# SciLifeLab/TIDDIT

Measured on AMD Instinct MI355X. Metric: cov bins/sec, 30x WGS synthetic (signals clustered/sec: see 'dbscan'), higher is better.
Workload: dtype int64; 1 GPU; BASELINE configs[1]: coverage histogram, 24 contigs x 125000000 bp (3.00 Gb), 30x 150-bp sorted stream, 500-bp bins, q>=20 filter; contigs split over the 1 rank(s); reads=600000000, bins=6000000

## Files before the change

### tiddit_amd/csrc/tdt_coverage.hip

```cpp
extern const char *const tdt_variant_coverage;
const char *const tdt_variant_coverage = ""
#ifdef COV_MIN_WAVES
    " COV_MIN_WAVES"
#endif
#ifdef COV_MIN_WAVES1
    " COV_MIN_WAVES1"
#endif
#ifdef COV_MIN_WAVES1_4
    " COV_MIN_WAVES1_4"
#endif
#ifdef COV_MIN_WAVES4
    " COV_MIN_WAVES4"
#endif
#ifdef COV_RPL
    " COV_RPL"
#endif
#ifdef COV_RPL1
    " COV_RPL1"
#endif
#ifdef COV_SPARES1
    " COV_SPARES1"
#endif
#ifdef COV_WIN
    " COV_WIN"
#endif
#ifdef COV_WIN1
    " COV_WIN1"
#endif
    ;

#include "tdt_common.h"

#include <algorithm>
#include <thread>

#define COV_THREADS 256
#ifndef COV_RPL
#define COV_RPL 8
#endif
#ifndef COV_RPL1
#define COV_RPL1 4
#endif
#define COV_READS_PER_BLOCK 16384
#ifndef COV_WIN
#define COV_WIN 2048
#endif
#define COV_LUT_LDS_MAX 1024
#define COV_PUSH_CHUNK (4u << 20)
#define COV_STATUS_BYTES (128 + COV_KEPT_SLOTS * 128)
#define COV_KEPT_SLOTS 512

struct CovItem {
    const int32_t *start;
    const int32_t *end;
    const uint8_t *mapq;
    const uint16_t *flag;
    const unsigned long long *packed;
    unsigned long long n;
    unsigned long long *acc;
    const unsigned long long *lut_end;
    int nbins;
    int aligned;
    unsigned first_block;
    unsigned binned;
};

struct CovParams {
    CovItem it;
    const CovItem *items;
    int n_items;
    int bin_size;
    unsigned magic;
    int shift;
    int min_q;
    int margin;
    unsigned xmax, m15;
    int k15;
    const unsigned long long *lut_main;
    unsigned long long one;
    int *status;
    unsigned long long *kept;
};

__device__ __forceinline__ int cov_div(int x, unsigned magic, int shift) {
    return shift < 0 ? x : (int)(__umulhi((unsigned)x, magic) >> shift);
}

#define DPP_WAVE_SHL1 0x130
#define DPP_WAVE_SHR1 0x138

template <int CTRL>
__device__ __forceinline__ unsigned long long dpp_u64(unsigned long long v) {
    const unsigned lo = __builtin_amdgcn_update_dpp(0u, (unsigned)v, CTRL, 0xf, 0xf, true);
    const unsigned hi = __builtin_amdgcn_update_dpp(0u, (unsigned)(v >> 32), CTRL, 0xf, 0xf, true);
    return ((unsigned long long)hi << 32) | lo;
}

#define COV_DPP_SHR1 "row_shr:1 row_mask:0xf bank_mask:0xf bound_ctrl:0"
#define COV_DPP_SHR2 "row_shr:2 row_mask:0xf bank_mask:0xf bound_ctrl:0"
#define COV_DPP_SHR4 "row_shr:4 row_mask:0xf bank_mask:0xf bound_ctrl:0"
#define COV_DPP_SHR8 "row_shr:8 row_mask:0xf bank_mask:0xf bound_ctrl:0"
#define COV_DPP_BC15 "row_bcast:15 row_mask:0xa bank_mask:0xf"
#define COV_DPP_BC31 "row_bcast:31 row_mask:0xc bank_mask:0xf"
#define COV_SCAN_ALL(STEP) \
    "s_nop 1\n\t" STEP(COV_DPP_SHR1) STEP(COV_DPP_SHR2) STEP(COV_DPP_SHR4) STEP(COV_DPP_SHR8) STEP(COV_DPP_BC15) STEP(COV_DPP_BC31) "s_nop 1"
#define COV_SCAN_STEP(CTRL)                                                                     \
    "v_add_co_u32_dpp %0, vcc, %0, %0 " CTRL "\n\t"                                             \
    "v_addc_co_u32_dpp %1, vcc, %1, %1, vcc " CTRL "\n\t"                                       \
    "v_add_co_u32_dpp %2, vcc, %2, %2 " CTRL "\n\t"                                             \
    "v_addc_co_u32_dpp %3, vcc, %3, %3, vcc " CTRL "\n\t"                                       \
    "v_add_co_u32_dpp %4, vcc, %4, %4 " CTRL "\n\t"                                             \
    "v_addc_co_u32_dpp %5, vcc, %5, %5, vcc " CTRL "\n\t"

__device__ __forceinline__ void wave_scan3_u64(unsigned long long &a0, unsigned long long &a1, unsigned long long &a2) {
    unsigned l0 = (unsigned)a0, h0 = (unsigned)(a0 >> 32), l1 = (unsigned)a1, h1 = (unsigned)(a1 >> 32),
             l2 = (unsigned)a2, h2 = (unsigned)(a2 >> 32);
    asm volatile(COV_SCAN_ALL(COV_SCAN_STEP) : "+v"(l0), "+v"(h0), "+v"(l1), "+v"(h1), "+v"(l2), "+v"(h2)::"vcc", "memory");
    a0 = ((unsigned long long)h0 << 32) | l0;
    a1 = ((unsigned long long)h1 << 32) | l1;
    a2 = ((unsigned long long)h2 << 32) | l2;
}

__device__ __forceinline__ unsigned long long cov_mask_lt(unsigned a, unsigned lim_uniform) {
    unsigned long long m;
    asm("v_cmp_gt_u32_e64 %0, %1, %2" : "=s"(m) : "s"(lim_uniform), "v"(a));
    return m;
}
__device__ __forceinline__ unsigned long long cov_mask_eq0(unsigned a) {
    unsigned long long m;
    asm("v_cmp_eq_u32_e64 %0, 0, %1" : "=s"(m) : "v"(a));
    return m;
}
__device__ __forceinline__ unsigned long long cov_mask_ne0(unsigned a) {
    unsigned long long m;
    asm("v_cmp_ne_u32_e64 %0, 0, %1" : "=s"(m) : "v"(a));
    return m;
}
__device__ __forceinline__ unsigned cov_select(unsigned long long m, unsigned if_set, unsigned if_clear) {
    unsigned r;
    asm("v_cndmask_b32_e64 %0, %1, %2, %3" : "=v"(r) : "v"(if_clear), "v"(if_set), "s"(m));
    return r;
}

#define COV_SCAN2_STEP(CTRL)                                                                    \
    "v_add_co_u32_dpp %0, vcc, %0, %0 " CTRL "\n\t"                                             \
    "v_addc_co_u32_dpp %1, vcc, %1, %1, vcc " CTRL "\n\t"                                       \
    "v_add_co_u32_dpp %2, vcc, %2, %2 " CTRL "\n\t"                                             \
    "v_addc_co_u32_dpp %3, vcc, %3, %3, vcc " CTRL "\n\t"

__device__ __forceinline__ void wave_scan2_u64(unsigned long long &a0, unsigned long long &a1) {
    unsigned l0 = (unsigned)a0, h0 = (unsigned)(a0 >> 32), l1 = (unsigned)a1, h1 = (unsigned)(a1 >> 32);
    asm volatile(COV_SCAN_ALL(COV_SCAN2_STEP) : "+v"(l0), "+v"(h0), "+v"(l1), "+v"(h1)::"vcc", "memory");
    a0 = ((unsigned long long)h0 << 32) | l0;
    a1 = ((unsigned long long)h1 << 32) | l1;
}

#define COV_SCAN4I_STEP(CTRL)                                                                   \
    "v_add_u32_dpp %0, %0, %0 " CTRL "\n\t"                                                     \
    "v_add_u32_dpp %1, %1, %1 " CTRL "\n\t"                                                     \
    "v_add_u32_dpp %2, %2, %2 " CTRL "\n\t"                                                     \
    "v_add_u32_dpp %3, %3, %3 " CTRL "\n\t"

__device__ __forceinline__ void wave_scan4_i32(int &p0, int &p1, int &p2, int &p3) {
    asm volatile(COV_SCAN_ALL(COV_SCAN4I_STEP) : "+v"(p0), "+v"(p1), "+v"(p2), "+v"(p3)::"memory");
}
// ... 75 lines not shown
            t.mq[j / 4] |= (ok ? (unsigned)P.mapq[idx + j] : 0u) << (8 * (j & 3));
            t.fl[j / 2] |= (ok ? (unsigned)P.flag[idx + j] : 0x4u) << (16 * (j & 1));
        }
    }
    return t;
}

template <int RPL>
struct CovTileP {
    unsigned long long w[RPL];
};

template <int RPL>
__device__ __forceinline__ CovTileP<RPL> cov_load_packed(const CovItem &P, unsigned long long idx, unsigned long long r1) {
    CovTileP<RPL> t;
    if (P.aligned && idx + RPL <= r1) {
#pragma unroll
        for (int k = 0; k < RPL / 2; k++) {
            const ulonglong2 v = *reinterpret_cast<const ulonglong2 *>(P.packed + idx + 2 * k);
            t.w[2 * k] = v.x;
            t.w[2 * k + 1] = v.y;
        }
    } else {
#pragma unroll
        for (int j = 0; j < RPL; j++) t.w[j] = idx + j < r1 ? P.packed[idx + j] : (1ull << 62);
    }
    return t;
}

__global__ void cov_pack(const int32_t *__restrict__ start, const int32_t *__restrict__ end, const uint8_t *__restrict__ mapq,
                         const uint16_t *__restrict__ flag, unsigned long long n, unsigned long long *__restrict__ out) {
    unsigned long long i = (unsigned long long)blockIdx.x * blockDim.x + threadIdx.x;
    const unsigned long long stride = (unsigned long long)gridDim.x * blockDim.x;
    for (; i < n; i += stride) out[i] = cov_pack_record(start[i], end[i], mapq[i], flag[i]);
}

__global__ void cov_pack_binned(const int32_t *__restrict__ start, const int32_t *__restrict__ end, const uint8_t *__restrict__ mapq,
                                const uint16_t *__restrict__ flag, unsigned long long n, int nbins, unsigned z, unsigned magic, int shift, int mode1,
                                unsigned long long *__restrict__ out) {
    unsigned long long i = (unsigned long long)blockIdx.x * blockDim.x + threadIdx.x;
    const unsigned long long stride = (unsigned long long)gridDim.x * blockDim.x;
    for (; i < n; i += stride) out[i] = cov_bin_record(start[i], end[i], mapq[i], flag[i], nbins, z, magic, shift, mode1 != 0);
}

#define COV_DBIT 48
#define COV_LOWMASK ((1ull << COV_DBIT) - 1ull)
#ifndef COV_WIN1
#define COV_WIN1 2048
#endif
#define COV_DQMAX 256
#ifndef COV_SPARES1
#define COV_SPARES1 64
#endif

#ifndef COV_MIN_WAVES
#define COV_MIN_WAVES 4
#endif
#ifndef COV_MIN_WAVES4
#define COV_MIN_WAVES4 3
#endif
#ifndef COV_MIN_WAVES1
#define COV_MIN_WAVES1 6
#endif
#ifndef COV_MIN_WAVES1_4
#define COV_MIN_WAVES1_4 4
#endif
template <bool LDS_LUT, int MODE, bool Z1, int RPL, int REC>
__global__ __launch_bounds__(COV_THREADS, MODE == 1 ? (REC ? COV_MIN_WAVES1 : COV_MIN_WAVES1_4) : (REC ? COV_MIN_WAVES : COV_MIN_WAVES4)) void cov_accumulate(CovParams P) {
    constexpr bool PACKED = REC != 0;
    extern __shared__ __attribute__((aligned(16))) unsigned long long smem[];
    constexpr int WIN = MODE == 1 ? COV_WIN1 : COV_WIN;
    constexpr int TILE = COV_THREADS * RPL;
    int *s_wsum = reinterpret_cast<int *>(smem);
    int *s_tbin = s_wsum + 4;
    int *s_rtot = reinterpret_cast<int *>(smem + 12);
    unsigned long long *win = smem + 12 + (MODE == 1 ? 16 : 0);
    unsigned long long *lutS = win + WIN + (MODE == 1 ? COV_SPARES1 : 2);

    const int tid = threadIdx.x;
    const int lane = tid & 63;
    CovItem I = P.it;
    unsigned blk = blockIdx.x;
    if (P.n_items > 0) {
        int lo = 0, hi = P.n_items;
        while (hi - lo > 1) {
            const int mid = (lo + hi) >> 1;
            if (P.items[mid].first_block <= blk) lo = mid;
            else hi = mid;
        }
        I = P.items[lo];
        blk -= I.first_block;
    }
    const unsigned long long r0 = (unsigned long long)blk * COV_READS_PER_BLOCK;
    const unsigned long long r1 = min(I.n, r0 + COV_READS_PER_BLOCK);
    const unsigned z = (unsigned)P.bin_size;
    const int last_bin = I.nbins - 1;
    auto div = [&](int x) { return Z1 ? x : (int)(__umulhi((unsigned)x, P.magic) >> P.shift); };

    auto load_tile = [&](unsigned long long idx) {
        if constexpr (PACKED) return cov_load_packed<RPL>(I, idx, r1);
        else return cov_load<RPL>(I, idx, r1);
    };
    auto cur = load_tile(r0 + (unsigned long long)tid * RPL);

    for (int i = tid; i < WIN + 2; i += COV_THREADS) win[i] = 0;
    if (LDS_LUT) {
        for (unsigned i = tid; i <= z; i += COV_THREADS) {
            const unsigned long long v = P.lut_main[i];
            lutS[i] = v;
            lutS[i + z + 1] = I.lut_end[i];
            if (MODE == 0 && !Z1) {
                unsigned long long *pr = lutS + 2 * (z + 1);
                pr[2 * i] = v;
                pr[2 * i + 1] = 0;
                pr[2 * (z + 1) + 2 * i] = 0;
                pr[2 * (z + 1) + 2 * i + 1] = v;
            }
            if (MODE == 1) {
                unsigned long long *tabA = lutS + 2 * (z + 1), *tabB = tabA + (z + 1), *tabL = tabB + (z + 1);
                tabA[i] = v & 0xffffffffull;
                tabB[i] = v << 32;
                tabL[i] = v - (1ull << COV_DBIT);
                if (i == 0) tabL[z + 1] = 0;
            }
        }
    }
    auto bin_of_read = [&](unsigned long long idx) {
        if constexpr (REC == 2) return (int)((unsigned)I.packed[idx] >> 2);
        int s = PACKED ? (int)(unsigned)I.packed[idx] : I.start[idx];
        s = s < 0 ? 0 : s;
        const int b = div(s);
        return b < I.nbins ? b : I.nbins - 1;
    };
    if (tid < COV_READS_PER_BLOCK / TILE) {
        const unsigned long long tl = min(r0 + (unsigned long long)(tid + 1) * TILE, r1) - 1;
        s_tbin[tid] = bin_of_read(tl);
    }
    int base = bin_of_read(r0);
    __syncthreads();
    auto lut = [&](unsigned i) -> unsigned long long {
        if (LDS_LUT) return lutS[i];
        return i <= z ? P.lut_main[i] : I.lut_end[i - z - 1];
    };

    auto contribute = [&](int bin, unsigned long long v) {
        const unsigned off = (unsigned)(bin - base);
        if (off < (unsigned)WIN) atomicAdd(&win[off], v);
        else if ((unsigned)bin <= (unsigned)last_bin) cov_global_add(I.acc, bin, v);
    };

    auto slow_read = [&](int s, int e) {
        const int fb = div(s);
        const int eb = div(e - 1);
        if (fb == eb) {
            contribute(fb, lut((unsigned)(e - s)));
        } else {
            contribute(fb, lut((unsigned)(fb + 1) * z - (unsigned)s));
            const unsigned bl = (unsigned)(e - 1) - (unsigned)eb * z;
            contribute(eb, lut(eb < last_bin ? bl : bl + z + 1));
            for (int b = fb + 1; b < eb; b++) contribute(b, P.one);
        }
    };

    auto spill = [&]() {
        __syncthreads();
        if constexpr (MODE == 1) {
            constexpr int PER = WIN / COV_THREADS;
            static_assert(PER == 8 && COV_THREADS == 256, "the packed resolve is written for eight rows of 256 words");
            unsigned long long w[PER];
#pragma unroll
            for (int k = 0; k < PER; k++) w[k] = win[k * COV_THREADS + tid];
            int pk[PER / 2];
#pragma unroll
// ... 308 lines not shown
            const unsigned long long q0 = dpp_u64<DPP_WAVE_SHR1>(a0), q1 = dpp_u64<DPP_WAVE_SHR1>(a1), q2 = dpp_u64<DPP_WAVE_SHR1>(a2);
            if (Knext != K) {
                if (a0) contribute(K, a0);
                if (a1) contribute(K + 1, a1);
                if (a2) contribute(K + 2, a2);
            }
            if (Kprev != K && lane != 0) {
                if (q0) contribute(K, 0ull - q0);
                if (q1) contribute(K + 1, 0ull - q1);
                if (q2) contribute(K + 2, 0ull - q2);
            }
        } else {
            const unsigned long long *tabA = lutS + 2 * (z + 1), *tabL = tabA + 2 * (z + 1);
            const unsigned ko = (unsigned)(K - base);
            const bool safe = ko < (unsigned)(WIN - COV_DQMAX - 2) && K + COV_DQMAX + 2 <= last_bin;
            const unsigned kw = safe ? ko : 0u;
            unsigned d1 = 0, d2 = 0;
            unsigned long long vL[RPL];
            unsigned woff[RPL];
#pragma unroll
            for (int j = 0; j < RPL; j++) {
                const unsigned rs = (unsigned)sv[j] - Kz;
                const unsigned re1 = (unsigned)ev[j] - Kz;
                const unsigned len = re1 - rs;
                bool cand;
                if constexpr (PACKED) cand = (unsigned)(cur.w[j] >> 32) - ((unsigned)P.min_q << 24) < ((64u - (unsigned)P.min_q) << 24);
                else cand = ((fl[j] & FMASK) == 0) & ((int)mq[j] >= P.min_q);
                const bool fast = cand & safe & (rs < 2u * z) & (len - 1u < P.xmax) & (re1 <= P.xmax);
                nkept += fast ? 1u : 0u;
                slowmask |= (cand & !fast) ? (1u << j) : 0u;
                const bool r1_ = rs >= z;
                const unsigned dq = (__umul24(re1, P.m15) - P.m15) >> P.k15;
                const bool multi = fast & (dq != (r1_ ? 1u : 0u));
                const unsigned bf = min(len, (r1_ ? 2u * z : z) - rs);
                const unsigned long long vv = tabA[(fast ? bf : 0u) + (r1_ ? z + 1u : 0u)];
                a0 += (unsigned)vv;
                a1 += (unsigned)(vv >> 32);
                d1 += (multi & !r1_) ? 1u : 0u;
                d2 += (multi & r1_) ? 1u : 0u;
                const unsigned bl1 = re1 - __umul24(dq, z);
                vL[j] = tabL[multi ? bl1 - 1u : z + 1u];
                woff[j] = multi ? kw + dq : (unsigned)WIN;
            }
#pragma unroll
            for (int j = 0; j < RPL; j++) atomicAdd(&win[woff[j]], vL[j]);
            atomicAdd(&win[kw], a0);
            atomicAdd(&win[kw + 1], a1 + ((unsigned long long)d1 << COV_DBIT));
            atomicAdd(&win[kw + 2], (unsigned long long)d2 << COV_DBIT);
            if (slowmask) {
#pragma unroll
                for (int j = 0; j < RPL; j++)
                    if (slowmask & (1u << j)) {
                        const int s = sv[j], e = true_end(j);
                        if (s < 0 || e <= s || div(e - 1) > last_bin) bad = true;
                        else { nkept++; slow_read(s, e); }
                    }
            }
        }
        cur = nxt;
    }

    for (int d = 32; d > 0; d >>= 1) nkept += __shfl_down(nkept, d);
    nkept += nkept_s;
    if (lane == 0 && nkept)
        atomicAdd(P.kept + (size_t)((blockIdx.x * (COV_THREADS / 64) + (tid >> 6)) % COV_KEPT_SLOTS) * 16, (unsigned long long)nkept);
    if (bad) atomicOr(P.status, 1);

    spill();
}

__global__ void cov_finalize(const long long *__restrict__ acc, double *__restrict__ out, long long n, double inv_scale,
                             int *status) {
    long long i = (long long)blockIdx.x * blockDim.x + threadIdx.x;
    const long long stride = (long long)gridDim.x * blockDim.x;
    bool inexact = false;
    for (; i < n; i += stride) {
        const long long a = acc[i];
        if (a >= (1ll << 53) || a < 0) inexact = true;
        out[i] = (double)a * inv_scale;
    }
    if (inexact) atomicOr(status, 2);
}

struct tdt_cov {
    tdt_ctx *ctx = nullptr;
    int n_contigs = 0;
    int bin_size = 0;
    int S = 0;
    bool small_bins = false;
    unsigned xmax = 0, m15 = 0;
    int k15 = 0;
    unsigned magic = 0;
    int shift = 0;
    std::vector<int64_t> len, nbins, off;
    std::vector<int> end_bin_size;
    int64_t total_bins = 0;
    unsigned long long *d_acc = nullptr;
    unsigned long long *d_lut_main = nullptr;
    unsigned long long *d_lut_end = nullptr;
    int *d_status = nullptr;
    unsigned long long *d_kept = nullptr;
    int *d_nbins = nullptr;
    void *d_stage[2] = {nullptr, nullptr};
    void *h_stage[2] = {nullptr, nullptr};
    hipEvent_t slot_ev[2] = {nullptr, nullptr};
    int slot_used[2] = {0, 0};
    int next_slot = 0;
};

static bool build_lut(std::vector<unsigned long long> &lut, int bin_size, int den, int S) {
    const double scale = ldexp(1.0, S);
    for (int b = 0; b <= bin_size; b++) {
        volatile float q = (float)b / (float)den;
        double f = (double)q * scale;
        unsigned long long fx = (unsigned long long)f;
        if ((double)fx != f) return false;
        lut[b] = fx;
    }
    return true;
}

extern "C" int tdt_cov_create(tdt_ctx *ctx, const int64_t *contig_len, int n_contigs, int bin_size, tdt_cov **out) {
    if (!ctx || !contig_len || !out || n_contigs <= 0) {
        tdt_set_error("tdt_cov_create: bad argument");
        return TDT_E_ARG;
    }
    *out = nullptr;
    if (bin_size <= 0 || bin_size > (1 << 24)) {
        tdt_set_error("tdt_cov_create: bin_size %d outside [1, 2^24] (reference: float32 bases are exact only there)",
                      bin_size);
        return TDT_E_ARG;
    }
    TDT_HIP(hipSetDevice(ctx->device));
    tdt_cov *c = new tdt_cov();
    c->ctx = ctx;
    c->n_contigs = n_contigs;
    c->bin_size = bin_size;
    const int L = tdt_ceil_log2_u64((uint64_t)bin_size);
    c->S = 23 + L + 1;
    {
        const char *env = getenv("TIDDIT_COV_MODE");
        const bool can = bin_size >= 2 && c->S <= 31;
        c->small_bins = can;
        if (env && env[0] == '0') c->small_bins = false;
        if (bin_size >= 2 && bin_size + 1 <= COV_LUT_LDS_MAX) {
            c->k15 = 15 + L;
            c->m15 = (unsigned)(((1ull << c->k15) + (unsigned)bin_size - 1) / (unsigned)bin_size);
            const unsigned lim = (unsigned)COV_DQMAX * (unsigned)bin_size;
            c->xmax = lim < 32768u ? lim : 32768u;
            for (unsigned x = 0; x < 32768u; x++)
                if (((x * c->m15) >> c->k15) != x / (unsigned)bin_size) {
                    tdt_set_error("internal: 24-bit division self-check failed for d=%d x=%u", bin_size, x);
                    delete c;
                    return TDT_E_ARG;
                }
        }
    }
    if (L == 0) {
        c->shift = -1;
        c->magic = 0;
    } else {
        const unsigned __int128 num = (unsigned __int128)1 << (31 + L);
        const unsigned __int128 m = (num + (unsigned)bin_size - 1) / (unsigned)bin_size;
        c->magic = (unsigned)m;
        c->shift = L - 1;
        const int probes[] = {0, 1, bin_size - 1, bin_size, bin_size + 1, 2 * bin_size - 1, 2 * bin_size, 1000003,
                              0x3fffffff, 0x7ffffffe, 0x7fffffff};
        for (int x : probes) {
            if (x < 0) continue;
            const int q = (int)(((unsigned long long)(unsigned)x * c->magic) >> 32 >> c->shift);
            if (q != x / bin_size) {
                tdt_set_error("internal: magic division self-check failed for d=%d x=%d", bin_size, x);
                delete c;
                return TDT_E_ARG;
            }
        }
    }
    c->len.assign(contig_len, contig_len + n_contigs);
    c->nbins.resize(n_contigs);
    c->off.resize(n_contigs);
    c->end_bin_size.resize(n_contigs);
    int64_t total = 0;
    for (int i = 0; i < n_contigs; i++) {
        const int64_t LN = contig_len[i];
        if (LN < 0 || LN > 0x7fffffffll) {
            tdt_set_error("tdt_cov_create: contig %d length %lld outside [0, 2^31)", i, (long long)LN);
            delete c;
            return TDT_E_ARG;
        }
        const int64_t bins = (LN + bin_size - 1) / bin_size;
        c->nbins[i] = bins;
        c->end_bin_size[i] = (int)(LN - (bins - 1) * bin_size);
        c->off[i] = total;
        total += bins;
        total = (total + 1) & ~1ll;
    }
    c->total_bins = total;
    const size_t lut_n = (size_t)bin_size + 1;
    std::vector<unsigned long long> lut(lut_n), lute((size_t)n_contigs * lut_n);
    if (!build_lut(lut, bin_size, bin_size, c->S)) {
        tdt_set_error("internal: fixed-point scale 2^-%d cannot represent float32(b)/float32(%d)", c->S, bin_size);
        delete c;
        return TDT_E_ARG;
    }
    for (int i = 0; i < n_contigs; i++) {
        std::vector<unsigned long long> t(lut_n);
        const int ebs = c->end_bin_size[i] > 0 ? c->end_bin_size[i] : bin_size;
        const double scale = ldexp(1.0, c->S);
        for (size_t b = 0; b < lut_n; b++) {
            volatile float q = (float)b / (float)ebs;
            double f = (double)q * scale;
            unsigned long long fx = (f < 9007199254740992.0) ? (unsigned long long)f : 0ull;
            t[b] = (f < 9007199254740992.0 && (double)fx == f) ? fx : (1ull << 53);
        }
        memcpy(&lute[(size_t)i * lut_n], t.data(), lut_n * sizeof(unsigned long long));
    }
    hipError_t e;
    auto fail = [&](const char *what) {
        tdt_set_error("tdt_cov_create: %s failed: %s", what, hipGetErrorString(e));
        tdt_cov_destroy(c);
        return TDT_E_HIP;
    };
    if ((e = tdt_dev_malloc((void **)&c->d_acc, (size_t)(total > 0 ? total : 1) * 8)) != hipSuccess) return fail("hipMalloc(acc)");
    if ((e = tdt_dev_malloc((void **)&c->d_lut_main, lut_n * 8)) != hipSuccess) return fail("hipMalloc(lut)");
    if ((e = tdt_dev_malloc((void **)&c->d_lut_end, (size_t)n_contigs * lut_n * 8)) != hipSuccess) return fail("hipMalloc(lut_end)");
    if ((e = tdt_dev_malloc((void **)&c->d_status, COV_STATUS_BYTES)) != hipSuccess) return fail("hipMalloc(status)");
    {
        std::vector<int> nb32(c->nbins.begin(), c->nbins.end());
        if ((e = tdt_dev_malloc((void **)&c->d_nbins, (size_t)n_contigs * 4)) != hipSuccess) return fail("hipMalloc(nbins)");
        if ((e = hipMemcpy(c->d_nbins, nb32.data(), (size_t)n_contigs * 4, hipMemcpyHostToDevice)) != hipSuccess) return fail("hipMemcpy(nbins)");
    }
    c->d_kept = (unsigned long long *)((char *)c->d_status + 128);
    if ((e = hipMemcpy(c->d_lut_main, lut.data(), lut_n * 8, hipMemcpyHostToDevice)) != hipSuccess) return fail("hipMemcpy(lut)");
    if ((e = hipMemcpy(c->d_lut_end, lute.data(), (size_t)n_contigs * lut_n * 8, hipMemcpyHostToDevice)) != hipSuccess)
        return fail("hipMemcpy(lut_end)");
    if ((e = hipMemset(c->d_acc, 0, (size_t)(total > 0 ? total : 1) * 8)) != hipSuccess) return fail("hipMemset(acc)");
    if ((e = hipMemset(c->d_status, 0, COV_STATUS_BYTES)) != hipSuccess) return fail("hipMemset(status)");
    for (int i = 0; i < 2; i++)
        if ((e = hipEventCreateWithFlags(&c->slot_ev[i], hipEventDisableTiming)) != hipSuccess) return fail("hipEventCreate");
    *out = c;
    return TDT_OK;
}

extern "C" void tdt_cov_destroy(tdt_cov *c) {
    if (!c) return;
    (void)hipSetDevice(c->ctx->device);
    (void)hipStreamSynchronize(c->ctx->stream);
    if (c->d_acc) (void)hipFree(c->d_acc);
    if (c->d_lut_main) (void)hipFree(c->d_lut_main);
    if (c->d_lut_end) (void)hipFree(c->d_lut_end);
    if (c->d_status) (void)hipFree(c->d_status);
    if (c->d_nbins) (void)hipFree(c->d_nbins);
    for (int i = 0; i < 2; i++) {
        if (c->d_stage[i]) (void)hipFree(c->d_stage[i]);
        if (c->h_stage[i]) (void)hipHostFree(c->h_stage[i]);
        if (c->slot_ev[i]) (void)hipEventDestroy(c->slot_ev[i]);
    }
    delete c;
}

extern "C" int tdt_cov_nbins(tdt_cov *c, int tid, int64_t *nbins, int *end_bin_size) {
    if (!c || tid < 0 || tid >= c->n_contigs) {
        tdt_set_error("tdt_cov_nbins: bad contig id");
        return TDT_E_ARG;
    }
    if (nbins) *nbins = c->nbins[tid];
    if (end_bin_size) *end_bin_size = c->end_bin_size[tid];
    return TDT_OK;
}

extern "C" int tdt_cov_scale_bits(tdt_cov *c) { return c ? c->S : TDT_E_ARG; }

extern "C" int tdt_cov_reset(tdt_cov *c) {
    if (!c) return TDT_E_ARG;
    TDT_HIP(hipSetDevice(c->ctx->device));
    TDT_HIP(hipMemsetAsync(c->d_acc, 0, (size_t)(c->total_bins > 0 ? c->total_bins : 1) * 8, c->ctx->stream));
    TDT_HIP(hipMemsetAsync(c->d_status, 0, COV_STATUS_BYTES, c->ctx->stream));
    return TDT_OK;
}

static CovItem cov_item(tdt_cov *c, int tid, const int32_t *d_start, const int32_t *d_end, const uint8_t *d_mapq,
                        const uint16_t *d_flag, size_t n) {
    CovItem it;
    it.start = d_start;
    it.end = d_end;
    it.mapq = d_mapq;
    it.flag = d_flag;
    it.packed = nullptr;
    it.n = n;
    it.acc = c->d_acc + c->off[tid];
    it.lut_end = c->d_lut_end + (size_t)tid * ((size_t)c->bin_size + 1);
    it.nbins = (int)c->nbins[tid];
    it.aligned = (((uintptr_t)d_start | (uintptr_t)d_end) & 15) == 0 && ((uintptr_t)d_mapq & (COV_RPL - 1)) == 0 &&
                 ((uintptr_t)d_flag & (2 * COV_RPL - 1)) == 0;
    it.first_block = 0;
    it.binned = 0;
    return it;
}

static CovItem cov_item_packed(tdt_cov *c, int tid, const unsigned long long *d_packed, const int32_t *d_end, size_t n) {
    CovItem it = cov_item(c, tid, nullptr, d_end, nullptr, nullptr, n);
    it.packed = d_packed;
    it.aligned = ((uintptr_t)d_packed & 15) == 0;
    return it;
}

static int cov_launch_items(tdt_cov *c, const CovItem &single, const CovItem *d_items, int n_items, unsigned grid, int min_q) {
    CovParams P;
    P.it = single;
    P.items = d_items;
    P.n_items = n_items;
    P.bin_size = c->bin_size;
    P.magic = c->magic;
    P.shift = c->shift;
    P.min_q = min_q;
    P.lut_main = c->d_lut_main;
    P.one = 1ull << c->S;
    P.status = c->d_status;
    P.kept = c->d_kept;
    const bool small = c->small_bins;
    P.margin = small ? COV_DQMAX + 8 : 640 / c->bin_size + 4;
    P.xmax = c->xmax;
    P.m15 = c->m15;
    P.k15 = c->k15;
    const bool lds_lut = c->bin_size + 1 <= COV_LUT_LDS_MAX;
    const size_t lds = 96 + (small ? 128 : 0) + ((size_t)(small ? COV_WIN1 + COV_SPARES1 : COV_WIN + 2)) * 8 + (lds_lut ? 2 * ((size_t)c->bin_size + 1) * 8 : 0) +
                       (small ? (3 * ((size_t)c->bin_size + 1) + 1) * 8 : 0) + ((!small && lds_lut && c->shift >= 0) ? 4 * ((size_t)c->bin_size + 1) * 8 : 0);
    const bool packed = single.packed != nullptr;
    const bool binned = packed && single.binned;
    if (binned && small)
        hipLaunchKernelGGL((cov_accumulate<true, 1, false, COV_RPL1, 2>), dim3(grid), dim3(COV_THREADS), lds, c->ctx->stream, P);
    else if (binned)
        hipLaunchKernelGGL((cov_accumulate<true, 0, false, COV_RPL, 2>), dim3(grid), dim3(COV_THREADS), lds, c->ctx->stream, P);
    else if (small && packed)
        hipLaunchKernelGGL((cov_accumulate<true, 1, false, COV_RPL1, 1>), dim3(grid), dim3(COV_THREADS), lds, c->ctx->stream, P);
    else if (small)
        hipLaunchKernelGGL((cov_accumulate<true, 1, false, COV_RPL1, 0>), dim3(grid), dim3(COV_THREADS), lds, c->ctx->stream, P);
    else if (lds_lut && c->shift >= 0 && packed)
        hipLaunchKernelGGL((cov_accumulate<true, 0, false, COV_RPL, 1>), dim3(grid), dim3(COV_THREADS), lds, c->ctx->stream, P);
    else if (lds_lut && c->shift >= 0)
        hipLaunchKernelGGL((cov_accumulate<true, 0, false, COV_RPL, 0>), dim3(grid), dim3(COV_THREADS), lds, c->ctx->stream, P);
    else if (lds_lut && packed)
        hipLaunchKernelGGL((cov_accumulate<true, 0, true, COV_RPL, 1>), dim3(grid), dim3(COV_THREADS), lds, c->ctx->stream, P);
    else if (lds_lut)
        hipLaunchKernelGGL((cov_accumulate<true, 0, true, COV_RPL, 0>), dim3(grid), dim3(COV_THREADS), lds, c->ctx->stream, P);
    else if (packed)
        hipLaunchKernelGGL((cov_accumulate<false, 0, false, COV_RPL, 1>), dim3(grid), dim3(COV_THREADS), lds, c->ctx->stream, P);
    else
        hipLaunchKernelGGL((cov_accumulate<false, 0, false, COV_RPL, 0>), dim3(grid), dim3(COV_THREADS), lds, c->ctx->stream, P);
    TDT_CHECK_LAUNCH();
    return TDT_OK;
}

static int cov_launch(tdt_cov *c, int tid, const int32_t *d_start, const int32_t *d_end, const uint8_t *d_mapq,
                      const uint16_t *d_flag, size_t n, int min_q) {
    if (n == 0 || c->nbins[tid] == 0) return TDT_OK;
    const unsigned grid = (unsigned)((n + COV_READS_PER_BLOCK - 1) / COV_READS_PER_BLOCK);
    return cov_launch_items(c, cov_item(c, tid, d_start, d_end, d_mapq, d_flag, n), nullptr, 0, grid, min_q);
}

extern "C" int tdt_cov_push_device_multi(tdt_cov *c, int n_items, const int *tids, const int32_t *const *d_start,
                                         const int32_t *const *d_end, const uint8_t *const *d_mapq,
                                         const uint16_t *const *d_flag, const size_t *n, int min_q) {
    if (!c || n_items < 0 || (n_items && (!tids || !d_start || !d_end || !d_mapq || !d_flag || !n))) {
        tdt_set_error("tdt_cov_push_device_multi: bad argument");
        return TDT_E_ARG;
    }
    TDT_HIP(hipSetDevice(c->ctx->device));
    std::vector<CovItem> items;
    unsigned long long blocks = 0;
    for (int i = 0; i < n_items; i++) {
        if (tids[i] < 0 || tids[i] >= c->n_contigs || (n[i] && (!d_start[i] || !d_end[i] || !d_mapq[i] || !d_flag[i]))) {
            tdt_set_error("tdt_cov_push_device_multi: bad item %d", i);
            return TDT_E_ARG;
        }
        if (n[i] == 0 || c->nbins[tids[i]] == 0) continue;
        CovItem it = cov_item(c, tids[i], d_start[i], d_end[i], d_mapq[i], d_flag[i], n[i]);
        it.first_block = (unsigned)blocks;
        blocks += (n[i] + COV_READS_PER_BLOCK - 1) / COV_READS_PER_BLOCK;
        items.push_back(it);
    }
    if (items.empty()) return TDT_OK;
    if (blocks >= 0x7fffffffull) {
        tdt_set_error("tdt_cov_push_device_multi: too many reads for one launch");
        return TDT_E_ARG;
    }
    void *d_items = nullptr;
    int rc = tdt_scratch(c->ctx, 7, items.size() * sizeof(CovItem), &d_items);
    if (rc) return rc;
    TDT_HIP(hipMemcpyAsync(d_items, items.data(), items.size() * sizeof(CovItem), hipMemcpyHostToDevice, c->ctx->stream));
    return cov_launch_items(c, items[0], (const CovItem *)d_items, (int)items.size(), (unsigned)blocks, min_q);
}

extern "C" int tdt_cov_pack_device(tdt_ctx *ctx, const int32_t *d_start, const int32_t *d_end, const uint8_t *d_mapq, const uint16_t *d_flag,
                                   size_t n, uint64_t *d_packed) {
    if (!ctx || (n && (!d_start || !d_end || !d_mapq || !d_flag || !d_packed))) {
        tdt_set_error("tdt_cov_pack_device: bad argument");
        return TDT_E_ARG;
    }
    if (!n) return TDT_OK;
    TDT_HIP(hipSetDevice(ctx->device));
    size_t blocks = (n + 255) / 256;
    if (blocks > 65536) blocks = 65536;
    hipLaunchKernelGGL(cov_pack, dim3((unsigned)blocks), dim3(256), 0, ctx->stream, d_start, d_end, d_mapq, d_flag, (unsigned long long)n,
                       (unsigned long long *)d_packed);
    TDT_CHECK_LAUNCH();
    return TDT_OK;
}

extern "C" int tdt_cov_push_packed_device_multi(tdt_cov *c, int n_items, const int *tids, const uint64_t *const *d_packed,
                                                const int32_t *const *d_end, const size_t *n, int min_q) {
    if (!c || n_items < 0 || (n_items && (!tids || !d_packed || !n))) {
        tdt_set_error("tdt_cov_push_packed_device_multi: bad argument");
        return TDT_E_ARG;
    }
    if (min_q > 63) {
        tdt_set_error("tdt_cov_push_packed_device_multi: packed records keep min(mapq, 63); min_q %d needs the unpacked entry point", min_q);
        return TDT_E_UNSUPPORTED;
    }
    if (min_q < 0) min_q = 0;
    TDT_HIP(hipSetDevice(c->ctx->device));
    std::vector<CovItem> items;
    unsigned long long blocks = 0;
    for (int i = 0; i < n_items; i++) {
        if (tids[i] < 0 || tids[i] >= c->n_contigs || (n[i] && !d_packed[i])) {
            tdt_set_error("tdt_cov_push_packed_device_multi: bad item %d", i);
            return TDT_E_ARG;
        }
        if (n[i] == 0 || c->nbins[tids[i]] == 0) continue;
        CovItem it = cov_item_packed(c, tids[i], (const unsigned long long *)d_packed[i], d_end ? d_end[i] : nullptr, n[i]);
        it.first_block = (unsigned)blocks;
        blocks += (n[i] + COV_READS_PER_BLOCK - 1) / COV_READS_PER_BLOCK;
        items.push_back(it);
    }
    if (items.empty()) return TDT_OK;
    if (blocks >= 0x7fffffffull) {
        tdt_set_error("tdt_cov_push_packed_device_multi: too many reads for one launch");
        return TDT_E_ARG;
    }
    void *d_items = nullptr;
    int rc = tdt_scratch(c->ctx, 7, items.size() * sizeof(CovItem), &d_items);
    if (rc) return rc;
    TDT_HIP(hipMemcpyAsync(d_items, items.data(), items.size() * sizeof(CovItem), hipMemcpyHostToDevice, c->ctx->stream));
    return cov_launch_items(c, items[0], (const CovItem *)d_items, (int)items.size(), (unsigned)blocks, min_q);
}

int tdt_cov_bin_spec(tdt_cov *c, CovBinSpec *out) {
    *out = CovBinSpec();
    if (!c) return TDT_E_ARG;
    if (c->bin_size < 2 || c->bin_size + 1 > COV_LUT_LDS_MAX) return TDT_OK;
    out->z = (unsigned)c->bin_size;
    out->magic = c->magic;
    out->shift = c->shift;
    out->mode1 = c->small_bins ? 1 : 0;
    out->d_nbins = c->d_nbins;
    out->n_contigs = c->n_contigs;
    return TDT_OK;
}

extern "C" int tdt_cov_pack_binned_device(tdt_cov *c, int tid, const int32_t *d_start, const int32_t *d_end, const uint8_t *d_mapq,
                                          const uint16_t *d_flag, size_t n, uint64_t *d_binned) {
    if (!c || tid < 0 || tid >= c->n_contigs || (n && (!d_start || !d_end || !d_mapq || !d_flag || !d_binned))) {
        tdt_set_error("tdt_cov_pack_binned_device: bad argument");
        return TDT_E_ARG;
    }
    CovBinSpec sp;
    tdt_cov_bin_spec(c, &sp);
    if (!sp.z) {
        tdt_set_error("tdt_cov_pack_binned_device: binned records exist for 2 <= bin_size < 1024 (this histogram: %d)", c->bin_size);
        return TDT_E_UNSUPPORTED;
    }
    if (!n) return TDT_OK;
    TDT_HIP(hipSetDevice(c->ctx->device));
    size_t blocks = (n + 255) / 256;
    if (blocks > 65536) blocks = 65536;
    hipLaunchKernelGGL(cov_pack_binned, dim3((unsigned)blocks), dim3(256), 0, c->ctx->stream, d_start, d_end, d_mapq, d_flag, (unsigned long long)n,
                       (int)c->nbins[tid], sp.z, sp.magic, sp.shift, sp.mode1, (unsigned long long *)d_binned);
    TDT_CHECK_LAUNCH();
    return TDT_OK;
}

extern "C" int tdt_cov_push_binned_device_multi(tdt_cov *c, int n_items, const int *tids, const uint64_t *const *d_binned,
                                                const int32_t *const *d_start, const int32_t *const *d_end, const size_t *n, int min_q) {
    if (!c || n_items < 0 || (n_items && (!tids || !d_binned || !d_start || !d_end || !n))) {
        tdt_set_error("tdt_cov_push_binned_device_multi: bad argument");
        return TDT_E_ARG;
    }
    if (c->bin_size < 2 || c->bin_size + 1 > COV_LUT_LDS_MAX) {
        tdt_set_error("tdt_cov_push_binned_device_multi: binned records exist for 2 <= bin_size < 1024 (this histogram: %d)", c->bin_size);
        return TDT_E_UNSUPPORTED;
    }
    if (min_q > 63) {
        tdt_set_error("tdt_cov_push_binned_device_multi: records keep min(mapq, 63); min_q %d needs the unpacked entry point", min_q);
        return TDT_E_UNSUPPORTED;
    }
    if (min_q < 0) min_q = 0;
    TDT_HIP(hipSetDevice(c->ctx->device));
    std::vector<CovItem> items;
    unsigned long long blocks = 0;
    for (int i = 0; i < n_items; i++) {
        if (tids[i] < 0 || tids[i] >= c->n_contigs || (n[i] && (!d_binned[i] || !d_start[i] || !d_end[i]))) {
            tdt_set_error("tdt_cov_push_binned_device_multi: bad item %d (the literal path needs the start and end arrays)", i);
            return TDT_E_ARG;
        }
        if (n[i] == 0 || c->nbins[tids[i]] == 0) continue;
        CovItem it = cov_item_packed(c, tids[i], (const unsigned long long *)d_binned[i], d_end[i], n[i]);
        it.start = d_start[i];
        it.binned = 1;
        it.first_block = (unsigned)blocks;
        blocks += (n[i] + COV_READS_PER_BLOCK - 1) / COV_READS_PER_BLOCK;
        items.push_back(it);
    }
    if (items.empty()) return TDT_OK;
    if (blocks >= 0x7fffffffull) {
        tdt_set_error("tdt_cov_push_binned_device_multi: too many reads for one launch");
        return TDT_E_ARG;
    }
    void *d_items = nullptr;
    int rc = tdt_scratch(c->ctx, 7, items.size() * sizeof(CovItem), &d_items);
    if (rc) return rc;
    TDT_HIP(hipMemcpyAsync(d_items, items.data(), items.size() * sizeof(CovItem), hipMemcpyHostToDevice, c->ctx->stream));
    return cov_launch_items(c, items[0], (const CovItem *)d_items, (int)items.size(), (unsigned)blocks, min_q);
}

extern "C" int tdt_cov_push_device(tdt_cov *c, int tid, const int32_t *d_start, const int32_t *d_end,
                                   const uint8_t *d_mapq, const uint16_t *d_flag, size_t n, int min_q) {
    if (!c || tid < 0 || tid >= c->n_contigs || (n && (!d_start || !d_end || !d_mapq || !d_flag))) {
        tdt_set_error("tdt_cov_push_device: bad argument");
        return TDT_E_ARG;
    }
    TDT_HIP(hipSetDevice(c->ctx->device));
    return cov_launch(c, tid, d_start, d_end, d_mapq, d_flag, n, min_q);
}

extern "C" int tdt_cov_push(tdt_cov *c, int tid, const int32_t *start, const int32_t *end, const uint8_t *mapq,
                            const uint16_t *flag, size_t n, int min_q) {
    if (!c || tid < 0 || tid >= c->n_contigs || (n && (!start || !end || !mapq || !flag))) {
        tdt_set_error("tdt_cov_push: bad argument");
        return TDT_E_ARG;
    }
    TDT_HIP(hipSetDevice(c->ctx->device));
    const size_t chunk = COV_PUSH_CHUNK;
    const size_t slot_bytes = chunk * 12;
    for (size_t o = 0; o < n; o += chunk) {
        const size_t m = n - o < chunk ? n - o : chunk;
        const int s = c->next_slot;
        c->next_slot ^= 1;
        if (!c->h_stage[s]) {
            TDT_HIP(hipHostMalloc(&c->h_stage[s], slot_bytes, hipHostMallocDefault));
            TDT_HIP(tdt_dev_malloc(&c->d_stage[s], slot_bytes));
        }
        if (c->slot_used[s]) TDT_HIP(hipEventSynchronize(c->slot_ev[s]));
        char *h = (char *)c->h_stage[s];
        char *d = (char *)c->d_stage[s];
        const size_t o_end = chunk * 4, o_flag = chunk * 8, o_mapq = chunk * 10;
        if (m >= (1u << 18) && tdt_host_thread_count() >= 4) {
            std::thread t1([&] { memcpy(h, start + o, m * 4); });
            std::thread t2([&] { memcpy(h + o_end, end + o, m * 4); });
            std::thread t3([&] { memcpy(h + o_flag, flag + o, m * 2); });
            memcpy(h + o_mapq, mapq + o, m);
            t1.join();
            t2.join();
            t3.join();
        } else {
            memcpy(h, start + o, m * 4);
            memcpy(h + o_end, end + o, m * 4);
            memcpy(h + o_flag, flag + o, m * 2);
            memcpy(h + o_mapq, mapq + o, m);
        }
        if (m == chunk) {
            TDT_HIP(hipMemcpyAsync(d, h, chunk * 11, hipMemcpyHostToDevice, c->ctx->stream));
        } else {
            TDT_HIP(hipMemcpyAsync(d, h, m * 4, hipMemcpyHostToDevice, c->ctx->stream));
            TDT_HIP(hipMemcpyAsync(d + o_end, h + o_end, m * 4, hipMemcpyHostToDevice, c->ctx->stream));
            TDT_HIP(hipMemcpyAsync(d + o_flag, h + o_flag, m * 2, hipMemcpyHostToDevice, c->ctx->stream));
            TDT_HIP(hipMemcpyAsync(d + o_mapq, h + o_mapq, m, hipMemcpyHostToDevice, c->ctx->stream));
        }
        int rc = cov_launch(c, tid, (const int32_t *)d, (const int32_t *)(d + o_end), (const uint8_t *)(d + o_mapq),
                            (const uint16_t *)(d + o_flag), m, min_q);
        if (rc) return rc;
        TDT_HIP(hipEventRecord(c->slot_ev[s], c->ctx->stream));
        c->slot_used[s] = 1;
    }
    return TDT_OK;
}

static int cov_status(tdt_cov *c) {
    int st[4];
    TDT_HIP(hipMemcpyAsync(st, c->d_status, 16, hipMemcpyDeviceToHost, c->ctx->stream));
    TDT_HIP(hipStreamSynchronize(c->ctx->stream));
    if (st[0] & 1) {
        tdt_set_error("coverage: a read maps outside its contig's bins (reference raises IndexError) or has end <= start");
        return TDT_E_RANGE;
    }
    if (st[0] & 2) {
        tdt_set_error("coverage: a bin exceeded 2^53 fixed-point units; the float64 sum is no longer exact");
        return TDT_E_INEXACT;
    }
    return TDT_OK;
}

extern "C" int tdt_cov_finish_device(tdt_cov *c, int tid, double *d_out) {
    if (!c || tid < 0 || tid >= c->n_contigs || (!d_out && c->nbins[tid])) {
        tdt_set_error("tdt_cov_finish_device: bad argument");
        return TDT_E_ARG;
// ... 89 lines not shown
```

Measured before the change: 6.764 billion bins/s.

## Pass item descriptors inline in kernel args and fuse reset memsets into one kernel

Up to 32 item descriptors now travel inside the kernel-argument block, and the device reads them through the kernarg segment pointer. This removes the per-launch host-to-device copy of the item table from pageable memory. Larger tables are staged through a ring of pinned host buffers guarded by events. The reset path replaces two hipMemsetAsync calls with one clear kernel using 16-byte stores. The cost is a larger kernel-argument payload on every launch, and the clear assumes total_bins is even, since an odd count would leave the last bin uncleared.

Result: no change. 6.812 billion bins/s, median of 4 (+0.7%).

```diff
diff --git a/tiddit_amd/csrc/tdt_coverage.hip b/tiddit_amd/csrc/tdt_coverage.hip
--- a/tiddit_amd/csrc/tdt_coverage.hip
+++ b/tiddit_amd/csrc/tdt_coverage.hip
@@ -49,6 +49,8 @@
 #define COV_PUSH_CHUNK (4u << 20)
 #define COV_STATUS_BYTES (128 + COV_KEPT_SLOTS * 128)
 #define COV_KEPT_SLOTS 512
+#define COV_INLINE_ITEMS 32
+#define COV_DESC_SLOTS 4
 
 struct CovItem {
     const int32_t *start;
@@ -80,7 +82,9 @@
     unsigned long long one;
     int *status;
     unsigned long long *kept;
+    CovItem inl[COV_INLINE_ITEMS];
 };
+static_assert(sizeof(CovItem) == 80 && sizeof(CovParams) <= 3072, "the descriptors must fit the kernel-argument segment (4 KB) with room to spare");
 
 __device__ __forceinline__ int cov_div(int x, unsigned magic, int shift) {
     return shift < 0 ? x : (int)(__umulhi((unsigned)x, magic) >> shift);
@@ -322,13 +326,23 @@
     CovItem I = P.it;
     unsigned blk = blockIdx.x;
     if (P.n_items > 0) {
+#if defined(__HIP_DEVICE_COMPILE__)
+        typedef const CovItem __attribute__((address_space(1))) *cov_item_ptr;
+        typedef const char __attribute__((address_space(4))) *cov_arg_ptr;
+        const cov_item_ptr tab = P.items ? (cov_item_ptr)P.items
+                                         : (cov_item_ptr)((cov_arg_ptr)__builtin_amdgcn_kernarg_segment_ptr() + offsetof(CovParams, inl));
+#else
+        const CovItem *tab = P.items ? P.items : P.inl;
+#endif
         int lo = 0, hi = P.n_items;
         while (hi - lo > 1) {
             const int mid = (lo + hi) >> 1;
-            if (P.items[mid].first_block <= blk) lo = mid;
+            if (tab[mid].first_block <= blk) lo = mid;
             else hi = mid;
         }
-        I = P.items[lo];
+        I.start = tab[lo].start; I.end = tab[lo].end; I.mapq = tab[lo].mapq; I.flag = tab[lo].flag; I.packed = tab[lo].packed;
+        I.n = tab[lo].n; I.acc = tab[lo].acc; I.lut_end = tab[lo].lut_end; I.nbins = tab[lo].nbins; I.aligned = tab[lo].aligned;
+        I.first_block = tab[lo].first_block; I.binned = tab[lo].binned;
         blk -= I.first_block;
     }
     const unsigned long long r0 = (unsigned long long)blk * COV_READS_PER_BLOCK;
@@ -803,6 +817,14 @@
     if (inexact) atomicOr(status, 2);
 }
 
+__global__ __launch_bounds__(256) void cov_clear(uint4 *__restrict__ acc, size_t n_acc16, uint4 *__restrict__ status, size_t n_status16) {
+    const size_t stride = (size_t)gridDim.x * blockDim.x;
+    const size_t t = (size_t)blockIdx.x * blockDim.x + threadIdx.x;
+    const uint4 zero = make_uint4(0, 0, 0, 0);
+    for (size_t i = t; i < n_status16; i += stride) status[i] = zero;
+    for (size_t i = t; i < n_acc16; i += stride) acc[i] = zero;
+}
+
 struct tdt_cov {
     tdt_ctx *ctx = nullptr;
     int n_contigs = 0;
@@ -827,6 +849,11 @@
     hipEvent_t slot_ev[2] = {nullptr, nullptr};
     int slot_used[2] = {0, 0};
     int next_slot = 0;
+    CovItem *h_desc[COV_DESC_SLOTS] = {};
+    size_t desc_cap[COV_DESC_SLOTS] = {};
+    hipEvent_t desc_ev[COV_DESC_SLOTS] = {};
+    int desc_used[COV_DESC_SLOTS] = {};
+    int next_desc = 0;
 };
 
 static bool build_lut(std::vector<unsigned long long> &lut, int bin_size, int den, int S) {
@@ -959,6 +986,8 @@
     if ((e = hipMemset(c->d_status, 0, COV_STATUS_BYTES)) != hipSuccess) return fail("hipMemset(status)");
     for (int i = 0; i < 2; i++)
         if ((e = hipEventCreateWithFlags(&c->slot_ev[i], hipEventDisableTiming)) != hipSuccess) return fail("hipEventCreate");
+    for (int i = 0; i < COV_DESC_SLOTS; i++)
+        if ((e = hipEventCreateWithFlags(&c->desc_ev[i], hipEventDisableTiming)) != hipSuccess) return fail("hipEventCreate");
     *out = c;
     return TDT_OK;
 }
@@ -977,6 +1006,10 @@
         if (c->h_stage[i]) (void)hipHostFree(c->h_stage[i]);
         if (c->slot_ev[i]) (void)hipEventDestroy(c->slot_ev[i]);
     }
+    for (int i = 0; i < COV_DESC_SLOTS; i++) {
+        if (c->h_desc[i]) (void)hipHostFree(c->h_desc[i]);
+        if (c->desc_ev[i]) (void)hipEventDestroy(c->desc_ev[i]);
+    }
     delete c;
 }
 
@@ -995,8 +1028,13 @@
 extern "C" int tdt_cov_reset(tdt_cov *c) {
     if (!c) return TDT_E_ARG;
     TDT_HIP(hipSetDevice(c->ctx->device));
-    TDT_HIP(hipMemsetAsync(c->d_acc, 0, (size_t)(c->total_bins > 0 ? c->total_bins : 1) * 8, c->ctx->stream));
-    TDT_HIP(hipMemsetAsync(c->d_status, 0, COV_STATUS_BYTES, c->ctx->stream));
+    static_assert(COV_STATUS_BYTES % 16 == 0, "cov_clear stores 16 bytes at a time");
+    const size_t n_acc16 = (size_t)c->total_bins / 2, n_status16 = COV_STATUS_BYTES / 16;
+    size_t blocks = ((n_acc16 > n_status16 ? n_acc16 : n_status16) + 255) / 256;
+    const size_t cap = (size_t)c->ctx->num_cu * 8;
+    if (blocks > cap) blocks = cap;
+    hipLaunchKernelGGL(cov_clear, dim3((unsigned)blocks), dim3(256), 0, c->ctx->stream, (uint4 *)c->d_acc, n_acc16, (uint4 *)c->d_status, n_status16);
+    TDT_CHECK_LAUNCH();
     return TDT_OK;
 }
 
@@ -1026,11 +1064,34 @@
     return it;
 }
 
-static int cov_launch_items(tdt_cov *c, const CovItem &single, const CovItem *d_items, int n_items, unsigned grid, int min_q) {
+static int cov_launch_items(tdt_cov *c, const CovItem &single, const CovItem *h_items, int n_items, unsigned grid, int min_q) {
     CovParams P;
     P.it = single;
-    P.items = d_items;
+    P.items = nullptr;
     P.n_items = n_items;
+    if (n_items > 0 && n_items <= COV_INLINE_ITEMS) {
+        memcpy(P.inl, h_items, (size_t)n_items * sizeof(CovItem));
+    } else if (n_items > 0) {
+        const int s = c->next_desc;
+        c->next_desc = (s + 1) % COV_DESC_SLOTS;
+        if (c->desc_used[s]) TDT_HIP(hipEventSynchronize(c->desc_ev[s]));
+        if ((size_t)n_items > c->desc_cap[s]) {
+            if (c->h_desc[s]) TDT_HIP(hipHostFree(c->h_desc[s]));
+            c->h_desc[s] = nullptr;
+            c->desc_cap[s] = 0;
+            const size_t want = (size_t)n_items + (size_t)n_items / 4 + 256;
+            TDT_HIP(hipHostMalloc((void **)&c->h_desc[s], want * sizeof(CovItem), hipHostMallocDefault));
+            c->desc_cap[s] = want;
+        }
+        memcpy(c->h_desc[s], h_items, (size_t)n_items * sizeof(CovItem));
+        void *d_items = nullptr;
+        int rc = tdt_scratch(c->ctx, 7, (size_t)n_items * sizeof(CovItem), &d_items);
+        if (rc) return rc;
+        TDT_HIP(hipMemcpyAsync(d_items, c->h_desc[s], (size_t)n_items * sizeof(CovItem), hipMemcpyHostToDevice, c->ctx->stream));
+        TDT_HIP(hipEventRecord(c->desc_ev[s], c->ctx->stream));
+        c->desc_used[s] = 1;
+        P.items = (const CovItem *)d_items;
+    }
     P.bin_size = c->bin_size;
     P.magic = c->magic;
     P.shift = c->shift;
@@ -1106,11 +1167,7 @@
         tdt_set_error("tdt_cov_push_device_multi: too many reads for one launch");
         return TDT_E_ARG;
     }
-    void *d_items = nullptr;
-    int rc = tdt_scratch(c->ctx, 7, items.size() * sizeof(CovItem), &d_items);
-    if (rc) return rc;
-    TDT_HIP(hipMemcpyAsync(d_items, items.data(), items.size() * sizeof(CovItem), hipMemcpyHostToDevice, c->ctx->stream));
-    return cov_launch_items(c, items[0], (const CovItem *)d_items, (int)items.size(), (unsigned)blocks, min_q);
+    return cov_launch_items(c, items[0], items.data(), (int)items.size(), (unsigned)blocks, min_q);
 }
 
 extern "C" int tdt_cov_pack_device(tdt_ctx *ctx, const int32_t *d_start, const int32_t *d_end, const uint8_t *d_mapq, const uint16_t *d_flag,
@@ -1159,11 +1216,7 @@
         tdt_set_error("tdt_cov_push_packed_device_multi: too many reads for one launch");
         return TDT_E_ARG;
     }
-    void *d_items = nullptr;
-    int rc = tdt_scratch(c->ctx, 7, items.size() * sizeof(CovItem), &d_items);
-    if (rc) return rc;
-    TDT_HIP(hipMemcpyAsync(d_items, items.data(), items.size() * sizeof(CovItem), hipMemcpyHostToDevice, c->ctx->stream));
-    return cov_launch_items(c, items[0], (const CovItem *)d_items, (int)items.size(), (unsigned)blocks, min_q);
+    return cov_launch_items(c, items[0], items.data(), (int)items.size(), (unsigned)blocks, min_q);
 }
 
 int tdt_cov_bin_spec(tdt_cov *c, CovBinSpec *out) {
@@ -1237,11 +1290,7 @@
         tdt_set_error("tdt_cov_push_binned_device_multi: too many reads for one launch");
         return TDT_E_ARG;
     }
-    void *d_items = nullptr;
-    int rc = tdt_scratch(c->ctx, 7, items.size() * sizeof(CovItem), &d_items);
-    if (rc) return rc;
-    TDT_HIP(hipMemcpyAsync(d_items, items.data(), items.size() * sizeof(CovItem), hipMemcpyHostToDevice, c->ctx->stream));
-    return cov_launch_items(c, items[0], (const CovItem *)d_items, (int)items.size(), (unsigned)blocks, min_q);
+    return cov_launch_items(c, items[0], items.data(), (int)items.size(), (unsigned)blocks, min_q);
 }
 
 extern "C" int tdt_cov_push_device(tdt_cov *c, int tid, const int32_t *d_start, const int32_t *d_end,
```
